# google-deepmind/mujoco_warp

Hardware: NVIDIA H100
Metric: env-steps/sec (whole box) on humanoid.xml at nworld=8192 per GPU (higher is better)
Workload: dtype f32

## Files before the change

mujoco_warp_b200/csrc/k_position.cu:

```cuda

#include "mjb_math.cuh"
#include "mjb_team.cuh"
#include "mjb_types.cuh"

namespace {

struct PosLayout {
  int qpos, xpos, xquat, xipos, xanchor, xaxis, scom, cinert, cdof, buf, arena, gxpos, gxmat, M, total;
};

__host__ __device__ inline int pad4(int n) { return (n + 3) & ~3; }
__host__ __device__ inline PosLayout pos_layout(const ModelDev& m) {
  PosLayout L;
  int o = 0;
  auto take = [&](int n) { int r = o; o += pad4(n); return r; };
  L.xpos = take(3 * m.nbody); L.xquat = take(4 * m.nbody); L.xipos = take(3 * m.nbody);
  L.xanchor = take(3 * m.njnt); L.xaxis = take(3 * m.njnt); L.scom = take(3 * m.nbody);
  L.arena = take(pad4(m.nq) > pad4(9 * m.nbody) ? m.nq : 9 * m.nbody);
  L.qpos = L.arena;
  L.gxpos = L.xipos; L.gxmat = L.gxpos + pad4(3 * m.ngeom);
  L.buf = L.xpos; L.M = L.buf + pad4(6 * m.nv);
  if (o < L.gxmat + pad4(9 * m.ngeom)) o = L.gxmat + pad4(9 * m.ngeom);
  if (o < L.M + pad4(m.nC)) o = L.M + pad4(m.nC);
  L.cinert = take(10 * m.nbody); L.cdof = take(6 * m.nv);
// ... 44 lines not shown
    __syncwarp();
#pragma unroll 1
    for (int l = 1; l < m.nlevel; l++) {
#pragma unroll 1
      for (int i = m.level_adr[l] + sub; i < m.level_adr[l + 1]; i += LPW) {
        const int b = m.level_body[i], pid = m.body_parentid[b], jntadr = m.body_jntadr[b], jntnum = m.body_jntnum[b];
        if (jntnum == 1 && m.jnt_type[jntadr] == JNT_FREE) {
          const int qa = m.jnt_qposadr[jntadr];
          v3 p = ld3(qpos + qa);
          q4 q = qnormalize(ldq(qpos + qa + 3));
          st3(xpos + 3 * b, p); stq(xquat + 4 * b, q);
          st3(xanchor + 3 * jntadr, p); st3(xaxis + 3 * jntadr, ld3(m.jnt_axis + 3 * jntadr));
          continue;
        }
        q4 pq = ldq(xquat + 4 * pid);
        const int mc = m.nmocap > 0 ? m.body_mocapid[b] : -1;
        const v3 bpos = mc >= 0 ? ld3(d.mocap_pos + (wb * m.nmocap + mc) * 3) : ld3(m.body_pos + 3 * b);
        const q4 bquat = mc >= 0 ? ldq(d.mocap_quat + (wb * m.nmocap + mc) * 4) : ldq(m.body_quat + 4 * b);
        v3 pos = qrot(pq, bpos) + ld3(xpos + 3 * pid);
        q4 quat = qmul(pq, bquat);
#pragma unroll 1
        for (int j = jntadr; j < jntadr + jntnum; j++) {
          const int qa = m.jnt_qposadr[j], t = m.jnt_type[j];
          v3 jpos = ld3(m.jnt_pos + 3 * j), jax = ld3(m.jnt_axis + 3 * j);
          v3 anchor = qrot(quat, jpos) + pos, axis = qrot(quat, jax);
          if (t == JNT_BALL) {
            quat = qmul(quat, qnormalize(ldq(qpos + qa)));
            pos = anchor - qrot(quat, jpos);
          } else if (t == JNT_SLIDE) {
            pos = pos + axis * (qpos[qa] - m.qpos0[qa]);
          } else if (t == JNT_HINGE) {
            quat = qmul(quat, axis_angle_quat(jax, qpos[qa] - m.qpos0[qa]));
            pos = anchor - qrot(quat, jpos);
          }
          st3(xanchor + 3 * j, anchor); st3(xaxis + 3 * j, axis);
        }
        st3(xpos + 3 * b, pos); stq(xquat + 4 * b, qnormalize(quat));
      }
      __syncwarp();
    }
  }

  if (kin && m.ntendon > 0) {
#pragma unroll 1
    for (int t = valid ? sub : m.ntendon; t < m.ntendon; t += LPW) {
      d.ten_length[wb * m.ntendon + t] = tendon_length(m, t, qpos);
      for (int k = m.ten_J_rowadr[t]; k < m.ten_J_rowadr[t] + m.ten_J_rownnz[t]; k++) d.ten_J[wb * m.nJten + k] = m.ten_J0[k];
    }
  }

  if (mask & STG_TRANSMISSION) {
#pragma unroll 1
    for (int a = valid ? sub : m.nu; a < m.nu; a += LPW) {
      if (m.ntendon > 0 && m.actuator_trntype[a] == TRN_TENDON) {
        const int t = m.actuator_trnid[2 * a], adr = m.moment_rowadr0[a], nnz = m.moment_rownnz0[a], tadr = m.ten_J_rowadr[t];
        const float gear0 = m.actuator_gear[6 * a];
        d.actuator_length[wb * m.nu + a] = tendon_length(m, t, qpos) * gear0;
        d.moment_rownnz[wb * m.nu + a] = nnz;
        d.moment_rowadr[wb * m.nu + a] = adr;
        for (int k = 0; k < nnz; k++) {
          d.moment_colind[wb * m.nJmom + adr + k] = m.moment_colind0[adr + k];
          d.actuator_moment[wb * m.nJmom + adr + k] = m.ten_J0[tadr + k] * gear0;
        }
        continue;
      }
      const int j = m.actuator_trnid[2 * a], t = m.jnt_type[j], adr = m.moment_rowadr0[a], nnz = m.moment_rownnz0[a];
      const float* gear = m.actuator_gear + 6 * a;
      d.actuator_length[wb * m.nu + a] = (t == JNT_SLIDE || t == JNT_HINGE) ? qpos[m.jnt_qposadr[j]] * gear[0] : 0.f;
      d.moment_rownnz[wb * m.nu + a] = nnz;
      d.moment_rowadr[wb * m.nu + a] = adr;
#pragma unroll 1
      for (int k = 0; k < nnz; k++) {
        d.moment_colind[wb * m.nJmom + adr + k] = m.moment_colind0[adr + k];
        d.actuator_moment[wb * m.nJmom + adr + k] = gear[k];
      }
    }
  }

  __syncwarp();

  if (kin) {
#pragma unroll 2
    for (int b = sub; b < nb; b += LPW) {
      q4 q = ldq(xquat + 4 * b);
      quat_to_mat(q, xmat + 9 * b);
      st3(xipos + 3 * b, ld3(xpos + 3 * b) + qrot(q, ld3(m.body_ipos + 3 * b)));
    }
#pragma unroll 1
    for (int s = valid ? sub : m.nsite; s < m.nsite; s += LPW) {
      const int b = m.site_bodyid[s];
      q4 q = ldq(xquat + 4 * b);
      float mat[9];
      st3(d.site_xpos + (wb * m.nsite + s) * 3, ld3(xpos + 3 * b) + qrot(q, ld3(m.site_pos + 3 * s)));
      quat_to_mat(qmul(q, ldq(m.site_quat + 4 * s)), mat);
      for (int k = 0; k < 9; k++) d.site_xmat[(wb * m.nsite + s) * 9 + k] = mat[k];
    }
    st.store_fence();
    GSTORE(xpos, BLK(xpos), 3 * nb); GSTORE(xquat, BLK(xquat), 4 * nb); GSTORE(xmat, BLK(arena), 9 * nb); GSTORE(xipos, BLK(xipos), 3 * nb);
    GSTORE(xanchor, BLK(xanchor), 3 * nj); GSTORE(xaxis, BLK(xaxis), 3 * nj);
    st.store_commit();
    if (!com) {
      st.store_wait_read();
#pragma unroll 2
      for (int b = sub; b < nb; b += LPW) quat_to_mat(qmul(ldq(xquat + 4 * b), ldq(m.body_iquat + 4 * b)), ximat + 9 * b);
      st.store_fence();
      GSTORE(ximat, BLK(arena), 9 * nb);
      st.store_commit();
    }
  }
  __syncwarp();

  if (com) {
#pragma unroll 2
    for (int b = sub; b < nb; b += LPW) st3(scom + 3 * b, ld3(xipos + 3 * b) * m.body_mass[b]);
    __syncwarp();
#pragma unroll 1
    for (int l = m.nlevel - 2; l >= 0; l--) {
#pragma unroll 1
      for (int i = m.level_adr[l] + sub; i < m.level_adr[l + 1]; i += LPW) {
        const int b = m.level_body[i];
        v3 acc = ld3(scom + 3 * b);
        for (int c = m.body_childadr[b]; c < m.body_childadr[b + 1]; c++) acc = acc + ld3(scom + 3 * m.body_childid[c]);
        st3(scom + 3 * b, acc);
      }
      __syncwarp();
    }
#pragma unroll 2
    for (int b = sub; b < nb; b += LPW) {
      const float ms = m.body_subtreemass[b];
      if (ms != 0.f) st3(scom + 3 * b, ld3(scom + 3 * b) * (1.0f / ms));
    }
    __syncwarp();
    if (kin) st.store_wait_read();
#pragma unroll 2
    for (int b = sub; b < nb; b += LPW) {
      float* mat = ximat + 9 * b;
      quat_to_mat(qmul(ldq(xquat + 4 * b), ldq(m.body_iquat + 4 * b)), mat);
      const v3 inert = ld3(m.body_inertia + 3 * b);
      const float mass = m.body_mass[b];
      const v3 dif = ld3(xipos + 3 * b) - ld3(scom + 3 * m.body_rootid[b]);
      float* r = cinert + 10 * b;
      const float a0 = mat[0] * inert.x, a1 = mat[1] * inert.y, a2 = mat[2] * inert.z;
      const float b0 = mat[3] * inert.x, b1 = mat[4] * inert.y, b2 = mat[5] * inert.z;
      const float c0 = mat[6] * inert.x, c1 = mat[7] * inert.y, c2 = mat[8] * inert.z;
      r[0] = a0 * mat[0] + a1 * mat[1] + a2 * mat[2] + mass * (dif.y * dif.y + dif.z * dif.z);
      r[1] = b0 * mat[3] + b1 * mat[4] + b2 * mat[5] + mass * (dif.x * dif.x + dif.z * dif.z);
      r[2] = c0 * mat[6] + c1 * mat[7] + c2 * mat[8] + mass * (dif.x * dif.x + dif.y * dif.y);
      r[3] = a0 * mat[3] + a1 * mat[4] + a2 * mat[5] - mass * dif.x * dif.y;
      r[4] = a0 * mat[6] + a1 * mat[7] + a2 * mat[8] - mass * dif.x * dif.z;
      r[5] = b0 * mat[6] + b1 * mat[7] + b2 * mat[8] - mass * dif.y * dif.z;
      r[6] = mass * dif.x; r[7] = mass * dif.y; r[8] = mass * dif.z; r[9] = mass;
    }
#pragma unroll 2
    for (int j = sub; j < nj; j += LPW) {
      const int b = m.jnt_bodyid[j], t = m.jnt_type[j];
      int dof = m.jnt_dofadr[j];
      const v3 offset = ld3(scom + 3 * m.body_rootid[b]) - ld3(xanchor + 3 * j);
      if (t == JNT_FREE || t == JNT_BALL) {
        float xm[9];
        quat_to_mat(ldq(xquat + 4 * b), xm);
        if (t == JNT_FREE) {
          for (int k = 0; k < 18; k++) cdof[6 * dof + k] = 0.f;
          cdof[6 * dof + 3] = 1.f; cdof[6 * (dof + 1) + 4] = 1.f; cdof[6 * (dof + 2) + 5] = 1.f;
          dof += 3;
        }
        for (int k = 0; k < 3; k++) {
          v3 col = matcol(xm, k);
          st3(cdof + 6 * (dof + k), col); st3(cdof + 6 * (dof + k) + 3, cross(col, offset));
        }
      } else if (t == JNT_SLIDE) {
        st3(cdof + 6 * dof, mk3(0.f, 0.f, 0.f)); st3(cdof + 6 * dof + 3, ld3(xaxis + 3 * j));
      } else {
        v3 ax = ld3(xaxis + 3 * j);
        st3(cdof + 6 * dof, ax); st3(cdof + 6 * dof + 3, cross(ax, offset));
      }
    }
    st.store_fence();
    GSTORE(subtree_com, BLK(scom), 3 * nb); GSTORE(cinert, BLK(cinert), 10 * nb); GSTORE(cdof, BLK(cdof), 6 * nv);
    if (kin) GSTORE(ximat, BLK(arena), 9 * nb);
    st.store_commit();
  }
  __syncwarp();

  if (mask & STG_CAMLIGHT) {
#pragma unroll 1
    for (int c = valid ? sub : m.ncam; c < m.ncam; c += LPW) {
      const int mode = m.cam_mode[c], b = m.cam_bodyid[c], tb = m.cam_targetbodyid[c];
      const bool is_target = mode == CAM_TARGETBODY || mode == CAM_TARGETBODYCOM;
      v3 p; float mat[9];
      if (mode == CAM_TRACK) {
        for (int k = 0; k < 9; k++) mat[k] = m.cam_mat0[9 * c + k];
        p = ld3(xpos + 3 * b) + ld3(m.cam_pos0 + 3 * c);
      } else if (mode == CAM_TRACKCOM) {
        for (int k = 0; k < 9; k++) mat[k] = m.cam_mat0[9 * c + k];
        p = ld3(scom + 3 * b) + ld3(m.cam_poscom0 + 3 * c);
      } else if (is_target && tb >= 0) {
        q4 q = ldq(xquat + 4 * b);
        p = ld3(xpos + 3 * b) + qrot(q, ld3(m.cam_pos + 3 * c));
        v3 tp = mode == CAM_TARGETBODYCOM ? ld3(scom + 3 * tb) : ld3(xpos + 3 * tb);
        v3 m3 = normalize(p - tp), m1 = normalize(cross(mk3(0.f, 0.f, 1.f), m3)), m2 = normalize(cross(m3, m1));
        mat[0] = m1.x; mat[1] = m2.x; mat[2] = m3.x; mat[3] = m1.y; mat[4] = m2.y; mat[5] = m3.y; mat[6] = m1.z; mat[7] = m2.z; mat[8] = m3.z;
      } else {
        q4 q = ldq(xquat + 4 * b);
        p = ld3(xpos + 3 * b) + qrot(q, ld3(m.cam_pos + 3 * c));
        quat_to_mat(qmul(q, ldq(m.cam_quat + 4 * c)), mat);
      }
      st3(d.cam_xpos + (wb * m.ncam + c) * 3, p);
      for (int k = 0; k < 9; k++) d.cam_xmat[(wb * m.ncam + c) * 9 + k] = mat[k];
    }
#pragma unroll 1
    for (int l = valid ? sub : m.nlight; l < m.nlight; l += LPW) {
      const int mode = m.light_mode[l], b = m.light_bodyid[l], tb = m.light_targetbodyid[l];
      const bool is_target = mode == CAM_TARGETBODY || mode == CAM_TARGETBODYCOM;
      v3 p, dir;
      bool norm = true;
      q4 q = ldq(xquat + 4 * b);
      if (is_target && tb < 0) {
        p = ld3(xpos + 3 * b) + qrot(q, ld3(m.light_pos + 3 * l)); dir = qrot(q, ld3(m.light_dir + 3 * l)); norm = false;
      } else if (mode == CAM_TRACK) {
        dir = ld3(m.light_dir0 + 3 * l); p = ld3(xpos + 3 * b) + ld3(m.light_pos0 + 3 * l);
      } else if (mode == CAM_TRACKCOM) {
        dir = ld3(m.light_dir0 + 3 * l); p = ld3(scom + 3 * b) + ld3(m.light_poscom0 + 3 * l);
      } else if (is_target) {
        p = ld3(xpos + 3 * b) + qrot(q, ld3(m.light_pos + 3 * l));
        v3 tp = mode == CAM_TARGETBODYCOM ? ld3(scom + 3 * tb) : ld3(xpos + 3 * tb);
        dir = tp - p;
      } else {
        p = ld3(xpos + 3 * b) + qrot(q, ld3(m.light_pos + 3 * l)); dir = qrot(q, ld3(m.light_dir + 3 * l));
      }
      if (norm) dir = normalize(dir);
      st3(d.light_xpos + (wb * m.nlight + l) * 3, p);
      st3(d.light_xdir + (wb * m.nlight + l) * 3, dir);
    }
  }


  if (kin) {
    st.store_wait_read();
#pragma unroll 2
    for (int gi = sub; gi < ng; gi += LPW) {
      const int b = m.geom_bodyid[gi];
      if (m.body_weldid[b] == 0 && (m.nmocap == 0 || m.body_mocapid[m.body_rootid[b]] == -1)) {
        for (int k = 0; k < 3; k++) gxpos[3 * gi + k] = d.geom_xpos[(wb * ng + gi) * 3 + k];
        for (int k = 0; k < 9; k++) gxmat[9 * gi + k] = d.geom_xmat[(wb * ng + gi) * 9 + k];
      } else {
        q4 q = ldq(xquat + 4 * b);
        st3(gxpos + 3 * gi, ld3(xpos + 3 * b) + qrot(q, ld3(m.geom_pos + 3 * gi)));
        quat_to_mat(qmul(q, ldq(m.geom_quat + 4 * gi)), gxmat + 9 * gi);
      }
    }
    st.store_fence();
    GSTORE(geom_xpos, BLK(gxpos), 3 * ng); GSTORE(geom_xmat, BLK(gxmat), 9 * ng);
    st.store_commit();
  }

  if (crbm) {
    st.store_wait_read();
#pragma unroll 1
    for (int l = m.nlevel - 2; l >= 1; l--) {
#pragma unroll 1
      for (int i = m.level_adr[l] + sub; i < m.level_adr[l + 1]; i += LPW) {
        const int b = m.level_body[i];
        float acc[10];
#pragma unroll
        for (int k = 0; k < 10; k++) acc[k] = crb[10 * b + k];
#pragma unroll 1
        for (int c = m.body_childadr[b]; c < m.body_childadr[b + 1]; c++) {
          const float* cc = crb + 10 * m.body_childid[c];
#pragma unroll
          for (int k = 0; k < 10; k++) acc[k] += cc[k];
        }
#pragma unroll
        for (int k = 0; k < 10; k++) crb[10 * b + k] = acc[k];
      }
      __syncwarp();
    }
#pragma unroll 2
    for (int dd = sub; dd < nv; dd += LPW) inert_vec(crb + 10 * m.dof_bodyid[dd], cdof + 6 * dd, buf + 6 * dd);
    __syncwarp();
#pragma unroll 4
    for (int e = sub; e < m.nC; e += LPW) {
      const int i = m.M_entry_row[e], j = m.M_colind[e];
      float v = dot6(cdof + 6 * j, buf + 6 * i);
      if (i == j) v += m.dof_armature[i];
      Ms[e] = v;
    }
    st.store_fence();
    GSTORE(crb, BLK(cinert), 10 * nb); GSTORE(M, BLK(M), m.nC);
    st.store_commit();
  }
  st.store_wait_read();
#undef GLOAD
#undef GSTORE
#undef BLK
#undef ROW
}

}

static TeamKernel pos_kernel(const ModelDev& m, int lpw) {
  return m.batched ? k_position<32, true> : lpw == 8 ? k_position<8, false> : lpw == 16 ? k_position<16, false> : k_position<32, false>;
}

size_t smem_position(const ModelDev& m, const DataDev& d) { return team_shape(m, d.wn, pos_layout(m).total, pos_kernel).block_bytes; }
cudaError_t launch_position(const ModelDev& m, const DataDev& d, int mask, cudaStream_t s) { return team_launch(m, d, pos_layout(m).total, pos_kernel, mask, s); }
cudaError_t resident_worlds_position(const ModelDev& m, const DataDev& d, int* worlds, int* shape) {
  shape[3] = 0;
  return team_resident_worlds(m, d, pos_layout(m).total, pos_kernel, worlds, shape);
}
```

mujoco_warp_b200/csrc/k_velocity.cu:

```cuda

#include "mjb_fluid.cuh"
#include "mjb_math.cuh"
#include "mjb_team.cuh"
#include "mjb_types.cuh"

namespace {

struct VelLayout { int qvel, cdof, cinert, cvel, cdofdot, cacc, cfrc, qpas, qbias, qact, qsm, qld, x, af, total; };
__host__ __device__ inline VelLayout vel_layout(const ModelDev& m) {
  VelLayout L;
  int o = 0;
  auto pad = [](int n) { return (n + 3) & ~3; };
  auto take = [&](int n) { int r = o; o += pad(n); return r; };
  L.qpas = take(m.nv); L.qbias = take(m.nv);
  L.qsm = L.qpas; L.x = L.qbias;
  const int a0 = o;
  L.cdof = take(6 * m.nv); L.cinert = take(10 * m.nbody); L.qvel = take(m.nv);
  L.cvel = take(6 * m.nbody); L.cdofdot = take(6 * (m.nv > m.nbody ? m.nv : m.nbody)); L.cacc = take(6 * m.nbody);
  L.cfrc = L.cdofdot;
  if (pad(m.nv) + pad(m.nu) <= L.cvel - L.cinert) { L.qact = L.cinert; L.af = L.cinert + pad(m.nv); }
  else { L.qact = take(m.nv); L.af = take(m.nu); }
  L.qld = a0;
  if (o - a0 < pad(m.qld_total)) o = a0 + pad(m.qld_total);
  L.total = o;
  return L;
}

template <int LPW>
__device__ __forceinline__ void team_chol_upper(float* U, int n, float* x, bool solve, int sub) {
#pragma unroll 1
  for (int j = 0; j < n; j++) {
    const int iend = solve ? n + 1 : n;
#pragma unroll 1
    for (int i = j + sub; i < iend; i += LPW) {
      const bool rhs = i == n;
      const float* col = rhs ? x : U + i;
      const int cs = rhs ? 1 : n;
      float s0 = rhs ? x[j] : U[j * n + i], s1 = 0.f;
      int k = 0;
#pragma unroll 4
      for (; k + 1 < j; k += 2) {
        s0 -= U[k * n + j] * col[k * cs];
        s1 -= U[(k + 1) * n + j] * col[(k + 1) * cs];
      }
      if (k < j) s0 -= U[k * n + j] * col[k * cs];
      if (rhs) x[j] = s0 + s1; else U[j * n + i] = s0 + s1;
    }
    __syncwarp();
    const float piv = sqrtf(fmaxf(U[j * n + j], MJ_MINVAL)), inv = 1.0f / piv;
    __syncwarp();
#pragma unroll 1
    for (int i = j + sub; i < iend; i += LPW) {
      if (i == n) x[j] *= inv;
      else U[j * n + i] = i == j ? piv : U[j * n + i] * inv;
    }
    __syncwarp();
  }
  if (!solve) return;
#pragma unroll 1
  for (int j = n - 1; j >= 0; j--) {
    const float xj = x[j] / U[j * n + j];
    __syncwarp();
#pragma unroll 1
    for (int k = sub; k < j; k += LPW) x[k] -= U[k * n + j] * xj;
    if (sub == 0) x[j] = xj;
    __syncwarp();
  }
}

template <bool PEXT, int LPW, bool BAT>
__global__ void __launch_bounds__(256)
k_velocity(const __grid_constant__ ModelDev mp, const __grid_constant__ DataDev d, int mask) {
  constexpr bool FLUID = false;
  [[maybe_unused]] constexpr FluidDev f{};
#include "k_velocity_body.cuh"
}

template <int LPW, bool BAT>
__global__ void __launch_bounds__(256)
k_velocity_fluid(const __grid_constant__ ModelDev mp, const __grid_constant__ DataDev d, int mask, const __grid_constant__ FluidDev f) {
  constexpr bool PEXT = true, FLUID = true;
#include "k_velocity_body.cuh"
}

}

template <bool PEXT>
static TeamKernel vel_instance(int lpw, bool bat) {
  if (bat) return k_velocity<PEXT, 32, true>;
  return lpw == 8 ? k_velocity<PEXT, 8, false> : lpw == 16 ? k_velocity<PEXT, 16, false> : k_velocity<PEXT, 32, false>;
}
static bool vel_pext(const ModelDev& m) { return m.has_gravcomp || m.ntendon > 0; }
static TeamKernel vel_kernel(const ModelDev& m, int lpw) { return vel_pext(m) ? vel_instance<true>(lpw, m.batched) : vel_instance<false>(lpw, m.batched); }
using FluidKernel = void (*)(ModelDev, DataDev, int, FluidDev);
static FluidKernel vel_kernel_fluid(const ModelDev& m, int lpw) {
  if (m.batched) return k_velocity_fluid<32, true>;
  return lpw == 8 ? k_velocity_fluid<8, false> : lpw == 16 ? k_velocity_fluid<16, false> : k_velocity_fluid<32, false>;
}

size_t smem_velocity(const ModelDev& m, const DataDev& d, const FluidDev& f) {
  const int words = vel_layout(m).total;
  return f.has_fluid ? team_shape(m, d.wn, words, vel_kernel_fluid).block_bytes : team_shape(m, d.wn, words, vel_kernel).block_bytes;
}
cudaError_t launch_velocity(const ModelDev& m, const DataDev& d, int mask, cudaStream_t s, const FluidDev& f) {
  const int words = vel_layout(m).total;
  return f.has_fluid ? team_launch(m, d, words, vel_kernel_fluid, mask, s, f) : team_launch(m, d, words, vel_kernel, mask, s);
}
cudaError_t resident_worlds_velocity(const ModelDev& m, const DataDev& d, int* worlds, int* shape, const FluidDev& f) {
  const int words = vel_layout(m).total;
  shape[3] = f.has_fluid ? 2 : vel_pext(m) ? 1 : 0;
  return f.has_fluid ? team_resident_worlds(m, d, words, vel_kernel_fluid, worlds, shape) : team_resident_worlds(m, d, words, vel_kernel, worlds, shape);
}
```

mujoco_warp_b200/csrc/k_velocity_body.cuh:

```cuda
  extern __shared__ __align__(16) float smem[];
  constexpr int G = 32 / LPW;
  Team<LPW> T;
  T.init(d.w0, d.wn, d.nworld);
  if (T.nvalid <= 0) return;
  MJB_WORLD_MODEL(T.w)
  const int lane = T.lane, sub = T.sub, g = T.g, nval = T.nvalid;
  const bool valid = T.valid;
  const VelLayout L = vel_layout(mp);
  float* S = smem + (size_t)(threadIdx.x >> 5) * ((size_t)L.total * G + 4);
  Stager st;
  st.init(reinterpret_cast<uint64_t*>(S + (size_t)L.total * G), lane);
  const int nv = m.nv, nb = m.nbody, nu = m.nu;
#define FLD(f, n) (S + (size_t)L.f * G + (size_t)g * (n))
  float *qvel = FLD(qvel, nv), *cdof = FLD(cdof, 6 * nv), *cinert = FLD(cinert, 10 * nb), *cvel = FLD(cvel, 6 * nb), *cdofdot = FLD(cdofdot, 6 * nv),
        *cacc = FLD(cacc, 6 * nb), *cfrc = FLD(cfrc, 6 * nb), *q_passive = FLD(qpas, nv), *q_bias = FLD(qbias, nv), *q_act = FLD(qact, nv),
        *q_smooth = FLD(qsm, nv), *qld = FLD(qld, m.qld_total), *x = FLD(x, nv), *aforce = FLD(af, nu);
  const float* Mw = d.M + (size_t)T.w * m.nC;
#undef FLD
  const size_t wg = (size_t)T.wg0;
#define GLOAD(f, field, n) st.load(S + (size_t)L.f * G, d.field + wg * (size_t)(n), nval * (n))
#define GSTORE(field, f, n) st.store(d.field + wg * (size_t)(n), S + (size_t)L.f * G, nval * (n))
  const size_t wb = (size_t)T.w;
  const bool v_all = mask & STG_VELOCITY;

  GLOAD(qvel, qvel, nv); GLOAD(cdof, cdof, 6 * nv);
  if (v_all || (mask & STG_RNE)) GLOAD(cinert, cinert, 10 * nb);
  constexpr int MREG = 32;
  float mreg[MREG];
  const bool fac = mask & (STG_ACCELERATION | STG_FACTOR_ONLY);
#pragma unroll
  for (int k = 0; k < MREG; k++) { const int e = sub + k * LPW; mreg[k] = (fac && e < m.nC) ? Mw[e] : 0.f; }
  bool any_xfrc = false;
  if (mask & STG_ACCELERATION) {
#pragma unroll 4
    for (int i = sub; i < 6 * nb; i += LPW) any_xfrc |= d.xfrc_applied[wb * 6 * nb + i] != 0.f;
  }
  st.load_wait();

  if (mask & (STG_VELOCITY | STG_COMVEL | STG_PASSIVE | STG_RNE)) {
    if (v_all)
#pragma unroll 1
    for (int a = valid ? sub : nu; a < nu; a += LPW) {
      const int nnz = d.moment_rownnz[wb * nu + a], adr = d.moment_rowadr[wb * nu + a];
      float vel = 0.f;
      for (int k = 0; k < nnz; k++) vel += d.actuator_moment[wb * m.nJmom + adr + k] * qvel[d.moment_colind[wb * m.nJmom + adr + k]];
      d.actuator_velocity[wb * nu + a] = vel;
    }
    if (PEXT && v_all && m.ntendon > 0) {
#pragma unroll 1
      for (int t = valid ? sub : m.ntendon; t < m.ntendon; t += LPW) {
        float vel = 0.f;
        for (int k = m.ten_J_rowadr[t]; k < m.ten_J_rowadr[t] + m.ten_J_rownnz[t]; k++) vel += m.ten_J0[k] * qvel[m.ten_J_colind[k]];
        d.ten_velocity[wb * m.ntendon + t] = vel;
      }
    }
    if (v_all || (mask & STG_COMVEL)) {
    if (sub < 6) cvel[sub] = 0.f;
    __syncwarp();
#pragma unroll 1
    for (int l = 1; l < m.nlevel; l++) {
#pragma unroll 1
      for (int i = m.level_adr[l] + sub; i < m.level_adr[l + 1]; i += LPW) {
        const int b = m.level_body[i], pid = m.body_parentid[b], jntadr = m.body_jntadr[b], jntnum = m.body_jntnum[b];
        int dof = m.body_dofadr[b];
        float cv[6];
#pragma unroll
        for (int k = 0; k < 6; k++) cv[k] = cvel[6 * pid + k];
#pragma unroll 1
        for (int j = jntadr; j < jntadr + jntnum; j++) {
          const int t = m.jnt_type[j];
          if (t == JNT_FREE) {
            for (int q = 0; q < 3; q++) { const float v = qvel[dof + q]; for (int k = 0; k < 6; k++) { cv[k] += cdof[6 * (dof + q) + k] * v; cdofdot[6 * (dof + q) + k] = 0.f; } }
            for (int q = 3; q < 6; q++) motion_cross(cv, cdof + 6 * (dof + q), cdofdot + 6 * (dof + q));
            for (int q = 3; q < 6; q++) { const float v = qvel[dof + q]; for (int k = 0; k < 6; k++) cv[k] += cdof[6 * (dof + q) + k] * v; }
            dof += 6;
          } else if (t == JNT_BALL) {
            for (int q = 0; q < 3; q++) motion_cross(cv, cdof + 6 * (dof + q), cdofdot + 6 * (dof + q));
            for (int q = 0; q < 3; q++) { const float v = qvel[dof + q]; for (int k = 0; k < 6; k++) cv[k] += cdof[6 * (dof + q) + k] * v; }
            dof += 3;
          } else {
            motion_cross(cv, cdof + 6 * dof, cdofdot + 6 * dof);
            const float v = qvel[dof];
            for (int k = 0; k < 6; k++) cv[k] += cdof[6 * dof + k] * v;
            dof += 1;
          }
        }
#pragma unroll
        for (int k = 0; k < 6; k++) cvel[6 * b + k] = cv[k];
      }
      __syncwarp();
    }
    st.store_fence();
    GSTORE(cvel, cvel, 6 * nb); GSTORE(cdof_dot, cdofdot, 6 * nv);
    st.store_commit();
    } else if (mask & STG_RNE) {
      GLOAD(cvel, cvel, 6 * nb); GLOAD(cdofdot, cdof_dot, 6 * nv);
      st.load_wait();
    }

    if (v_all || (mask & STG_PASSIVE)) {
      const bool dsbl_spring = m.disableflags & DSBL_SPRING, dsbl_damper = m.disableflags & DSBL_DAMPER;
      const bool gravcomp = PEXT && m.has_gravcomp && !(m.disableflags & DSBL_GRAVITY) && !(dsbl_spring && dsbl_damper);
      [[maybe_unused]] const bool fluid = FLUID && !(dsbl_spring && dsbl_damper);
      if constexpr (FLUID) if (fluid) {
        const float* cv = (v_all || (mask & STG_COMVEL)) ? cvel : d.cvel + wb * 6 * nb;
        const float *xip = d.xipos + wb * nb * 3, *stc = d.subtree_com + wb * nb * 3;
#pragma unroll 1
        for (int b = sub; b < nb; b += LPW)
          fluid_body_wrench(m, f, b, cv + 6 * b, ld3(xip + 3 * b), d.ximat + (wb * nb + b) * 9, ld3(stc + 3 * m.body_rootid[b]), d.geom_xpos + wb * m.ngeom * 3,
                            d.geom_xmat + wb * m.ngeom * 9, cacc + 6 * b);
        __syncwarp();
      }
#pragma unroll 1
      for (int dd = sub; dd < nv; dd += LPW) {
        const int j = m.dof_jntid[dd], t = m.jnt_type[j];
        float spring = 0.f, damper = 0.f, gc = 0.f;
        if (!(dsbl_spring && dsbl_damper)) {
          const float stiffness = m.jnt_stiffness[j];
          if (stiffness != 0.f && !dsbl_spring) {
            const int qa = m.jnt_qposadr[j], k = dd - m.jnt_dofadr[j];
            if (t == JNT_SLIDE || t == JNT_HINGE) spring = -(d.qpos[wb * m.nq + qa] - m.qpos_spring[qa]) * stiffness;
            else if (!PEXT) {}
            else if (t == JNT_FREE && k < 3) spring = -stiffness * (d.qpos[wb * m.nq + qa + k] - m.qpos_spring[qa + k]);
            else {
              const int ra = t == JNT_FREE ? qa + 3 : qa, kk = t == JNT_FREE ? k - 3 : k;
              const q4 rot = qnormalize(ldq(d.qpos + wb * m.nq + ra)), ref = ldq(m.qpos_spring + ra);
              const q4 qd = qmul(mkq(ref.w, -ref.x, -ref.y, -ref.z), rot);
              const float s2 = sqrtf(qd.x * qd.x + qd.y * qd.y + qd.z * qd.z);
              if (s2 != 0.f) {
                float speed = 2.0f * atan2f(s2, qd.w);
                if (speed > 3.14159265358979f) speed -= 2.0f * 3.14159265358979f;
                spring = -stiffness * (kk == 0 ? qd.x : kk == 1 ? qd.y : qd.z) * (speed / s2);
              }
            }
          }
          const float damping = m.dof_damping[dd];
          if (damping != 0.f && !dsbl_damper) damper = -qvel[dd] * damping;
          if (PEXT && m.ntendon > 0) {
#pragma unroll 1
            for (int tn = 0; tn < m.ntendon; tn++) {
              const float ks = m.tendon_stiffness[tn], kd = m.tendon_damping[tn];
              if ((ks == 0.f || dsbl_spring) && (kd == 0.f || dsbl_damper)) continue;
              const float J = tendon_J_at(m, tn, dd);
              if (J == 0.f) continue;
              if (ks != 0.f && !dsbl_spring) {
                const float len = d.ten_length[wb * m.ntendon + tn], lo = m.tendon_lengthspring[2 * tn], hi = m.tendon_lengthspring[2 * tn + 1];
                const float x = len > hi ? len - hi : (len < lo ? len - lo : 0.f);
                spring += J * (-x * ks);
              }
              if (kd != 0.f && !dsbl_damper) {
                float vel = 0.f;
                for (int k = m.ten_J_rowadr[tn]; k < m.ten_J_rowadr[tn] + m.ten_J_rownnz[tn]; k++) vel += m.ten_J0[k] * qvel[m.ten_J_colind[k]];
                damper += J * (-vel * kd);
              }
            }
          }
        }
        if (gravcomp) {
#pragma unroll 1
          for (int b = 1; b < nb; b++) {
            const float g = m.body_gravcomp[b];
            if (g == 0.f || !m.body_isdofancestor[b * nv + dd]) continue;
            const float sc = -m.body_mass[b] * g;
            const v3 off = ld3(d.xipos + (wb * nb + b) * 3) - ld3(d.subtree_com + (wb * nb + m.body_rootid[b]) * 3);
            const v3 jp = ld3(cdof + 6 * dd + 3) + cross(ld3(cdof + 6 * dd), off);
            gc += sc * (jp.x * m.gravity_x + jp.y * m.gravity_y + jp.z * m.gravity_z);
          }
        }
        float passive = spring + damper + (m.jnt_actgravcomp[j] ? 0.f : gc);
        if constexpr (FLUID) {
          const float fl = fluid ? fluid_project(m, dd, cdof + 6 * dd, cacc, d.xipos + wb * nb * 3, d.subtree_com + wb * nb * 3) : 0.f;
          passive += fl;
          if (valid) f.qfrc_fluid[wb * nv + dd] = fl;
        }
        q_passive[dd] = passive;
        if (valid) {
          d.qfrc_spring[wb * nv + dd] = spring;
          d.qfrc_damper[wb * nv + dd] = damper;
          d.qfrc_gravcomp[wb * nv + dd] = gc;
          d.qfrc_passive[wb * nv + dd] = passive;
        }
      }
    }
    if (v_all || (mask & STG_RNE)) {
    for (int k = sub; k < 6; k += LPW) cacc[k] = k < 3 ? 0.f : ((m.disableflags & DSBL_GRAVITY) ? 0.f : -(k == 3 ? m.gravity_x : k == 4 ? m.gravity_y : m.gravity_z));
    __syncwarp();
#pragma unroll 1
    for (int l = 1; l < m.nlevel; l++) {
#pragma unroll 1
      for (int i = m.level_adr[l] + sub; i < m.level_adr[l + 1]; i += LPW) {
        const int b = m.level_body[i], pid = m.body_parentid[b];
        float a[6];
#pragma unroll
        for (int k = 0; k < 6; k++) a[k] = cacc[6 * pid + k];
#pragma unroll 1
        for (int q = 0; q < m.body_dofnum[b]; q++) {
          const int dof = m.body_dofadr[b] + q;
          const float v = qvel[dof];
#pragma unroll
          for (int k = 0; k < 6; k++) a[k] += cdofdot[6 * dof + k] * v;
        }
#pragma unroll
        for (int k = 0; k < 6; k++) cacc[6 * b + k] = a[k];
      }
      __syncwarp();
    }
    st.store_wait_read();
#pragma unroll 2
    for (int b = sub; b < nb; b += LPW) {
      float f[6] = {0.f, 0.f, 0.f, 0.f, 0.f, 0.f};
      if (b > 0) {
        float iv[6], g[6];
        inert_vec(cinert + 10 * b, cacc + 6 * b, f);
        inert_vec(cinert + 10 * b, cvel + 6 * b, iv);
        motion_cross_force(cvel + 6 * b, iv, g);
#pragma unroll
        for (int k = 0; k < 6; k++) f[k] += g[k];
      }
#pragma unroll
      for (int k = 0; k < 6; k++) cfrc[6 * b + k] = f[k];
    }
    __syncwarp();
#pragma unroll 1
    for (int l = m.nlevel - 2; l >= 0; l--) {
#pragma unroll 1
      for (int i = m.level_adr[l] + sub; i < m.level_adr[l + 1]; i += LPW) {
        const int b = m.level_body[i];
        float acc[6];
#pragma unroll
        for (int k = 0; k < 6; k++) acc[k] = cfrc[6 * b + k];
#pragma unroll 1
        for (int c = m.body_childadr[b]; c < m.body_childadr[b + 1]; c++) {
          const float* cc = cfrc + 6 * m.body_childid[c];
#pragma unroll
          for (int k = 0; k < 6; k++) acc[k] += cc[k];
        }
#pragma unroll
        for (int k = 0; k < 6; k++) cfrc[6 * b + k] = acc[k];
      }
      __syncwarp();
    }
#pragma unroll 1
    for (int dd = sub; dd < nv; dd += LPW) {
      const float v = dot6(cdof + 6 * dd, cfrc + 6 * m.dof_bodyid[dd]);
      q_bias[dd] = v;
    }
    st.store_fence();
    GSTORE(cacc, cacc, 6 * nb); GSTORE(cfrc_int, cfrc, 6 * nb); GSTORE(qfrc_bias, qbias, nv);
    st.store_commit();
    }
  } else if (mask & STG_ACCELERATION) {
    GLOAD(qpas, qfrc_passive, nv); GLOAD(qbias, qfrc_bias, nv);
    st.load_wait();
  }
  __syncwarp();

  if (mask & STG_ACTUATION) {
#pragma unroll 1
    for (int dd = sub; dd < nv; dd += LPW) q_act[dd] = 0.f;
    __syncwarp();
    const bool enabled = nu > 0 && !(m.disableflags & DSBL_ACTUATION);
#pragma unroll 1
    for (int a = sub; a < nu; a += LPW) {
      float force = 0.f;
      if (enabled) {
        float ctrl = d.ctrl[wb * nu + a];
        if (m.actuator_ctrllimited[a] && !(m.disableflags & DSBL_CLAMPCTRL)) ctrl = clampf(ctrl, m.actuator_ctrlrange[2 * a], m.actuator_ctrlrange[2 * a + 1]);
        const float length = d.actuator_length[wb * nu + a], velocity = d.actuator_velocity[wb * nu + a];
        const float *gp = m.actuator_gainprm + 10 * a, *bp = m.actuator_biasprm + 10 * a;
        float gain = 0.f, bias = 0.f;
        if (m.actuator_gaintype[a] == GAIN_FIXED) gain = gp[0];
        else if (m.actuator_gaintype[a] == GAIN_AFFINE) gain = gp[0] + gp[1] * length + gp[2] * velocity;
        if (m.actuator_biastype[a] == BIAS_AFFINE) bias = bp[0] + bp[1] * length + bp[2] * velocity;
        float ctrl_act = ctrl;
        if (m.na > 0 && m.actuator_actadr[a] >= 0) {
          const int last = m.actuator_actadr[a] + m.actuator_actnum[a] - 1, dyn = m.actuator_dyntype[a];
          const float act = d.act[wb * m.na + last];
          float act_dot = 0.f;
          if (dyn == DYN_INTEGRATOR) act_dot = ctrl;
          else if (dyn == DYN_FILTER || dyn == DYN_FILTEREXACT) act_dot = (ctrl - act) / fmaxf(m.actuator_dynprm[10 * a], MJ_MINVAL);
          if (valid) d.act_dot[wb * m.na + last] = act_dot;
          ctrl_act = m.actuator_actearly[a] ? next_act(m, a, act, act_dot, 1.0f, m.actuator_actlimited[a] != 0) : act;
        }
        force = gain * ctrl_act + bias;
        if (m.actuator_forcelimited[a]) force = clampf(force, m.actuator_forcerange[2 * a], m.actuator_forcerange[2 * a + 1]);
      } else if (m.na > 0 && m.actuator_actadr[a] >= 0 && valid) {
        d.act_dot[wb * m.na + m.actuator_actadr[a] + m.actuator_actnum[a] - 1] = 0.f;
      }
      if (valid) d.actuator_force[wb * nu + a] = force;
      aforce[a] = force;
    }
    __syncwarp();
    if (PEXT && enabled && m.ntendon > 0) {
#pragma unroll 1
      for (int t = sub; t < m.ntendon; t += LPW) {
        if (!m.tendon_actfrclimited[t]) continue;
        float total = 0.f;
        for (int b = 0; b < nu; b++) if (m.actuator_trntype[b] == TRN_TENDON && m.actuator_trnid[2 * b] == t) total += aforce[b];
        const float lo = m.tendon_actfrcrange[2 * t], hi = m.tendon_actfrcrange[2 * t + 1];
        const float sc = total < lo ? lo / total : (total > hi ? hi / total : 1.0f);
        if (sc == 1.0f) continue;
        for (int b = 0; b < nu; b++)
          if (m.actuator_trntype[b] == TRN_TENDON && m.actuator_trnid[2 * b] == t) { aforce[b] *= sc; if (valid) d.actuator_force[wb * nu + b] = aforce[b]; }
      }
      __syncwarp();
    }
    if (enabled) {
#pragma unroll 1
      for (int dd = sub; dd < nv; dd += LPW) {
        float q = 0.f;
        for (int k = m.dofact_adr[dd]; k < m.dofact_adr[dd + 1]; k++) q += d.actuator_moment[wb * m.nJmom + m.dofact_mom[k]] * aforce[m.dofact_act[k]];
        const int j = m.dof_jntid[dd];
        if (!(m.disableflags & DSBL_GRAVITY) && m.jnt_actgravcomp[j]) q += d.qfrc_gravcomp[wb * nv + dd];
        if (m.jnt_actfrclimited[j]) q = clampf(q, m.jnt_actfrcrange[2 * j], m.jnt_actfrcrange[2 * j + 1]);
        q_act[dd] = q;
      }
    }
    st.store_fence();
    GSTORE(qfrc_actuator, qact, nv);
    st.store_commit();
  } else if (mask & STG_ACCELERATION) {
    GLOAD(qact, qfrc_actuator, nv);
    st.load_wait();
  }
  __syncwarp();

  if (mask & (STG_ACCELERATION | STG_FACTOR_ONLY)) {
    if (mask & STG_ACCELERATION) {
#pragma unroll 1
      for (int dd = sub; dd < nv; dd += LPW) q_smooth[dd] = q_passive[dd] - q_bias[dd] + q_act[dd] + d.qfrc_applied[wb * nv + dd];
      if (team_any<LPW>(any_xfrc, g)) {
#pragma unroll 1
        for (int dd = sub; dd < nv; dd += LPW) {
          const float* cd = cdof + 6 * dd;
          const int db = m.dof_bodyid[dd];
          float acc = 0.f;
          for (int b = db; b < nb; b++) {
            const float* ft = d.xfrc_applied + (wb * nb + b) * 6;
            if (ft[0] == 0.f && ft[1] == 0.f && ft[2] == 0.f && ft[3] == 0.f && ft[4] == 0.f && ft[5] == 0.f) continue;
            int p = b;
            while (p != 0 && p != db) p = m.body_parentid[p];
            if (p == 0) continue;
            const v3 off = ld3(d.xipos + (wb * nb + b) * 3) - ld3(d.subtree_com + (wb * nb + m.body_rootid[b]) * 3);
            const v3 cr = cross(ld3(cd), off);
            acc += cd[3] * ft[0] + cd[4] * ft[1] + cd[5] * ft[2] + cd[0] * ft[3] + cd[1] * ft[4] + cd[2] * ft[5] + dot(cr, ld3(ft));
          }
          q_smooth[dd] += acc;
        }
      }
      __syncwarp();
    }
    const bool acc = mask & STG_ACCELERATION;
    st.store_wait_read();
#pragma unroll 1
    for (int i = sub; i < m.qld_total; i += LPW) qld[i] = 0.f;
    if (acc)
#pragma unroll 1
      for (int i = sub; i < nv; i += LPW) x[i] = q_smooth[i];
    __syncwarp();
#pragma unroll 1
    for (int t = 0; t < m.ntree; t++) {
      const int start = m.tree_dofadr[t], n = m.tree_dofnum[t];
      float* U = qld + m.tree_qLDadr[t];
      const int e0 = m.M_rowadr[start], e1 = m.M_rowadr[start + n - 1] + m.M_rownnz[start + n - 1];
#pragma unroll
      for (int k = 0; k < MREG; k++) {
        const int e = sub + k * LPW;
        if (e >= e0 && e < e1) U[(m.M_colind[e] - start) * n + (m.M_entry_row[e] - start)] = mreg[k];
      }
#pragma unroll 1
      for (int e = max(e0, MREG * LPW) + ((sub - max(e0, MREG * LPW)) % LPW + LPW) % LPW; e < e1; e += LPW)
        U[(m.M_colind[e] - start) * n + (m.M_entry_row[e] - start)] = Mw[e];
      __syncwarp();
      team_chol_upper<LPW>(U, n, x + start, acc, sub);
    }
    st.store_fence();
    if (acc) { GSTORE(qfrc_smooth, qsm, nv); GSTORE(qacc_smooth, x, nv); }
    GSTORE(qLD, qld, m.qld_total);
    st.store_commit();
  }
  st.store_wait_read();
#undef GLOAD
#undef GSTORE
```

mujoco_warp_b200/csrc/mjb_team.cuh:

```cuda
#pragma once
#include <algorithm>
#include <climits>
#include <cstdint>
#include <cuda_runtime.h>

#include "mjb_launch.cuh"
#include "mjb_math.cuh"
#include "mjb_types.cuh"

template <int LPW>
__device__ __forceinline__ float team_sum(float v) {
#pragma unroll
  for (int o = LPW / 2; o > 0; o >>= 1) v += __shfl_xor_sync(FULL_MASK, v, o);
  return v;
}
template <int LPW>
__device__ __forceinline__ int team_sum_i(int v) {
#pragma unroll
  for (int o = LPW / 2; o > 0; o >>= 1) v += __shfl_xor_sync(FULL_MASK, v, o);
  return v;
}
template <int LPW>
__device__ __forceinline__ bool team_any(bool p, int g) {
  const unsigned b = __ballot_sync(FULL_MASK, p);
  return LPW == 32 ? b != 0u : ((b >> (g * LPW)) & ((1u << (LPW & 31)) - 1u)) != 0u;
}

__device__ __forceinline__ uint32_t smem_u32(const void* p) { return (uint32_t)__cvta_generic_to_shared(p); }

struct Stager {
  uint64_t* bar;
  uint32_t phase;
  int lane;
  bool pending_store;

  __device__ __forceinline__ void init(uint64_t* b, int lane_) {
    bar = b; phase = 0; lane = lane_; pending_store = false;
    if (lane == 0) {
      asm volatile("mbarrier.init.shared::cta.b64 [%0], 1;" ::"r"(smem_u32(bar)) : "memory");
      asm volatile("fence.mbarrier_init.release.cluster;" ::: "memory");
    }
    __syncwarp();
  }
  static __device__ __forceinline__ bool bulk_ok(const void* g, const void* s, int nfloats) {
    return (((uintptr_t)g | (uintptr_t)smem_u32(s)) & 15u) == 0 && (nfloats & 3) == 0 && nfloats > 0;
  }
  __device__ __forceinline__ void load(float* s, const float* g, int n) {
    if (bulk_ok(g, s, n)) {
      if (lane == 0) {
        const uint32_t bytes = (uint32_t)n * 4u;
        asm volatile("mbarrier.expect_tx.relaxed.cta.shared::cta.b64 [%0], %1;" ::"r"(smem_u32(bar)), "r"(bytes) : "memory");
        asm volatile("cp.async.bulk.shared::cluster.global.mbarrier::complete_tx::bytes [%0], [%1], %2, [%3];" ::"r"(smem_u32(s)), "l"(g),
                     "r"(bytes), "r"(smem_u32(bar))
                     : "memory");
      }
    } else {
#pragma unroll 1
      for (int i = lane; i < n; i += 32) s[i] = g[i];
    }
  }
  __device__ __forceinline__ void load_wait() {
    if (lane == 0) asm volatile("mbarrier.arrive.shared::cta.b64 _, [%0];" ::"r"(smem_u32(bar)) : "memory");
    uint32_t ok = 0;
    while (!ok) {
      asm volatile("{\n .reg .pred p;\n mbarrier.try_wait.parity.shared::cta.b64 p, [%1], %2;\n selp.u32 %0, 1, 0, p;\n}" : "=r"(ok) : "r"(smem_u32(bar)), "r"(phase) : "memory");
    }
    phase ^= 1u;
    __syncwarp();
  }
  __device__ __forceinline__ void store_fence() {
    asm volatile("fence.proxy.async.shared::cta;" ::: "memory");
    __syncwarp();
  }
  __device__ __forceinline__ void store(float* g, const float* s, int n) {
    if (bulk_ok(g, s, n)) {
      if (lane == 0) {
        asm volatile("cp.async.bulk.global.shared::cta.bulk_group [%0], [%1], %2;" ::"l"(g), "r"(smem_u32(s)), "r"((uint32_t)n * 4u) : "memory");
        pending_store = true;
      }
    } else {
#pragma unroll 1
      for (int i = lane; i < n; i += 32) g[i] = s[i];
    }
  }
  __device__ __forceinline__ void store_commit() {
    if (lane == 0 && pending_store) asm volatile("cp.async.bulk.commit_group;" ::: "memory");
  }
  __device__ __forceinline__ void store_wait_read() {
    if (lane == 0 && pending_store) { asm volatile("cp.async.bulk.wait_group.read 0;" ::: "memory"); pending_store = false; }
    __syncwarp();
  }
};

using TeamKernel = void (*)(ModelDev, DataDev, int);
template <class K>
using TeamChooserOf = K (*)(const ModelDev& m, int lpw);

struct TeamShape { int lpw, wpb; size_t block_bytes; };
template <class K>
inline TeamShape team_shape(const ModelDev& m, int nworld, size_t world_words, TeamChooserOf<K> kernel_of) {
  constexpr size_t kBlockMax = 200 * 1024;
  auto bytes = [&](int lpw) { return (world_words * (size_t)(32 / lpw) + 4) * sizeof(float); };
  int lpw = 8;
  while (lpw < 32 && bytes(lpw) > kBlockMax / 2) lpw *= 2;
  int wpb = 2;
  if (m.batched && lpw < 32) {
    lpw = 32;
  } else {
    const SmLimits& sm = sm_limits();
    const long groups = (nworld + 32 / lpw - 1) / (32 / lpw);
    const int warp_regs = (kernel_regs(kernel_of(m, lpw)) * 32 + 255) & ~255;
    auto rounds = [&](int w) {
      long per_sm = (long)(sm.smem_per_sm / sm_block_bytes(bytes(lpw) * w));
      per_sm = std::min({per_sm, (long)sm.blocks, (long)(sm.warps / w)});
      if (warp_regs > 0) per_sm = std::min(per_sm, (long)(sm.regs / warp_regs / w));
      const long fit = per_sm * sm.sms, blocks = (groups + w - 1) / w;
      return fit > 0 ? (blocks + fit - 1) / fit : LONG_MAX;
    };
    for (int w : {1, 4})
      if (bytes(lpw) * w <= kBlockMax && rounds(w) < rounds(wpb)) wpb = w;
  }
  while (wpb > 1 && bytes(lpw) * wpb > kBlockMax) wpb--;
  return TeamShape{lpw, wpb, bytes(lpw) * wpb};
}

inline int team_carveout(size_t block_bytes) {
  const size_t per_sm = sm_limits().smem_per_sm, block = sm_block_bytes(block_bytes), fit = per_sm / block;
  const size_t pct = fit > 0 ? (100 * fit * block + per_sm - 1) / per_sm : 100;
  return pct < 100 ? (int)pct : (int)cudaSharedmemCarveoutMaxShared;
}

template <class K, class... A>
inline cudaError_t team_launch(const ModelDev& m, const DataDev& d, size_t world_words, TeamChooserOf<K> kernel_of, int mask, cudaStream_t s, const A&... extra) {
  const TeamShape t = team_shape(m, d.wn, world_words, kernel_of);
  const int G = 32 / t.lpw, ngroups = (d.wn + G - 1) / G, grid = (ngroups + t.wpb - 1) / t.wpb;
  return launch(kernel_of(m, t.lpw), grid, 32 * t.wpb, t.block_bytes, team_carveout(t.block_bytes), s, m, d, mask, extra...);
}

template <class K>
inline cudaError_t team_resident_worlds(const ModelDev& m, const DataDev& d, size_t world_words, TeamChooserOf<K> kernel_of, int* worlds, int* shape) {
  const TeamShape t = team_shape(m, d.wn, world_words, kernel_of);
  const K kern = kernel_of(m, t.lpw);
  int blocks = 0;
  cudaError_t e = launch_configure((const void*)kern, t.block_bytes, team_carveout(t.block_bytes));
  if (e == cudaSuccess) e = cudaOccupancyMaxActiveBlocksPerMultiprocessor(&blocks, kern, 32 * t.wpb, t.block_bytes);
  *worlds = blocks * t.wpb * (32 / t.lpw);
  shape[0] = t.lpw; shape[1] = t.wpb; shape[2] = (int)t.block_bytes;
  return e;
}

template <int LPW>
struct Team {
  static constexpr int G = 32 / LPW;
  int lane, sub, g;
  int wg0, nvalid;
  int w;
  bool valid;
  __device__ __forceinline__ void init(int w0, int wn, int nworld) {
    lane = threadIdx.x & 31; sub = lane % LPW; g = lane / LPW;
    wg0 = w0 + (blockIdx.x * (blockDim.x >> 5) + (threadIdx.x >> 5)) * G;
    const int wend = min(w0 + wn, nworld);
    nvalid = min(G, wend - wg0);
    valid = g < nvalid;
    w = wg0 + (valid ? g : nvalid - 1);
  }
};
```

Measured before the change: 20.71 million.

## Let velocity kernel pick wider lanes-per-world teams with shifted bulk copies

The launch shape search now considers wider lane-per-world teams (up to the model's max tree size) for the velocity kernel when they need no more scheduling rounds. It also sizes from the total world count instead of the per-launch slice. To keep bulk async copies usable when per-world blocks are not 16-byte aligned at two worlds per warp, shared buffers are offset to match global alignment, with shifted load/store helpers that handle the unaligned edges. The LPW=16 instantiation gets a tighter launch bound and a smaller register array for the mass matrix, trading register spills for occupancy.

Result: faster. 20.91 million (median of 6 runs) (+1.0%).

```diff
diff --git a/mujoco_warp_b200/csrc/k_position.cu b/mujoco_warp_b200/csrc/k_position.cu
--- a/mujoco_warp_b200/csrc/k_position.cu
+++ b/mujoco_warp_b200/csrc/k_position.cu
@@ -370,9 +370,9 @@
   return m.batched ? k_position<32, true> : lpw == 8 ? k_position<8, false> : lpw == 16 ? k_position<16, false> : k_position<32, false>;
 }
 
-size_t smem_position(const ModelDev& m, const DataDev& d) { return team_shape(m, d.wn, pos_layout(m).total, pos_kernel).block_bytes; }
-cudaError_t launch_position(const ModelDev& m, const DataDev& d, int mask, cudaStream_t s) { return team_launch(m, d, pos_layout(m).total, pos_kernel, mask, s); }
+size_t smem_position(const ModelDev& m, const DataDev& d) { return team_shape(m, d.nworld, pos_layout(m).total, pos_kernel, 0).block_bytes; }
+cudaError_t launch_position(const ModelDev& m, const DataDev& d, int mask, cudaStream_t s) { return team_launch(m, d, pos_layout(m).total, pos_kernel, 0, mask, s); }
 cudaError_t resident_worlds_position(const ModelDev& m, const DataDev& d, int* worlds, int* shape) {
   shape[3] = 0;
-  return team_resident_worlds(m, d, pos_layout(m).total, pos_kernel, worlds, shape);
-}
+  return team_resident_worlds(m, d, pos_layout(m).total, pos_kernel, 0, worlds, shape);
+}
diff --git a/mujoco_warp_b200/csrc/k_velocity.cu b/mujoco_warp_b200/csrc/k_velocity.cu
--- a/mujoco_warp_b200/csrc/k_velocity.cu
+++ b/mujoco_warp_b200/csrc/k_velocity.cu
@@ -69,7 +69,7 @@
 }
 
 template <bool PEXT, int LPW, bool BAT>
-__global__ void __launch_bounds__(256)
+__global__ void __launch_bounds__(256, LPW == 16 ? 4 : 2)
 k_velocity(const __grid_constant__ ModelDev mp, const __grid_constant__ DataDev d, int mask) {
   constexpr bool FLUID = false;
   [[maybe_unused]] constexpr FluidDev f{};
@@ -100,14 +100,14 @@
 
 size_t smem_velocity(const ModelDev& m, const DataDev& d, const FluidDev& f) {
   const int words = vel_layout(m).total;
-  return f.has_fluid ? team_shape(m, d.wn, words, vel_kernel_fluid).block_bytes : team_shape(m, d.wn, words, vel_kernel).block_bytes;
+  return f.has_fluid ? team_shape(m, d.nworld, words, vel_kernel_fluid, m.maxtree).block_bytes : team_shape(m, d.nworld, words, vel_kernel, m.maxtree).block_bytes;
 }
 cudaError_t launch_velocity(const ModelDev& m, const DataDev& d, int mask, cudaStream_t s, const FluidDev& f) {
   const int words = vel_layout(m).total;
-  return f.has_fluid ? team_launch(m, d, words, vel_kernel_fluid, mask, s, f) : team_launch(m, d, words, vel_kernel, mask, s);
+  return f.has_fluid ? team_launch(m, d, words, vel_kernel_fluid, m.maxtree, mask, s, f) : team_launch(m, d, words, vel_kernel, m.maxtree, mask, s);
 }
 cudaError_t resident_worlds_velocity(const ModelDev& m, const DataDev& d, int* worlds, int* shape, const FluidDev& f) {
   const int words = vel_layout(m).total;
   shape[3] = f.has_fluid ? 2 : vel_pext(m) ? 1 : 0;
-  return f.has_fluid ? team_resident_worlds(m, d, words, vel_kernel_fluid, worlds, shape) : team_resident_worlds(m, d, words, vel_kernel, worlds, shape);
+  return f.has_fluid ? team_resident_worlds(m, d, words, vel_kernel_fluid, m.maxtree, worlds, shape) : team_resident_worlds(m, d, words, vel_kernel, m.maxtree, worlds, shape);
 }
diff --git a/mujoco_warp_b200/csrc/k_velocity_body.cuh b/mujoco_warp_b200/csrc/k_velocity_body.cuh
--- a/mujoco_warp_b200/csrc/k_velocity_body.cuh
+++ b/mujoco_warp_b200/csrc/k_velocity_body.cuh
@@ -11,21 +11,22 @@
   Stager st;
   st.init(reinterpret_cast<uint64_t*>(S + (size_t)L.total * G), lane);
   const int nv = m.nv, nb = m.nbody, nu = m.nu;
-#define FLD(f, n) (S + (size_t)L.f * G + (size_t)g * (n))
+  const int wgi = T.wg0;
+#define BLK(f, n) (S + (size_t)L.f * G + team_shift<G>(wgi, n))
+#define FLD(f, n) (BLK(f, n) + (size_t)g * (n))
   float *qvel = FLD(qvel, nv), *cdof = FLD(cdof, 6 * nv), *cinert = FLD(cinert, 10 * nb), *cvel = FLD(cvel, 6 * nb), *cdofdot = FLD(cdofdot, 6 * nv),
         *cacc = FLD(cacc, 6 * nb), *cfrc = FLD(cfrc, 6 * nb), *q_passive = FLD(qpas, nv), *q_bias = FLD(qbias, nv), *q_act = FLD(qact, nv),
         *q_smooth = FLD(qsm, nv), *qld = FLD(qld, m.qld_total), *x = FLD(x, nv), *aforce = FLD(af, nu);
   const float* Mw = d.M + (size_t)T.w * m.nC;
-#undef FLD
   const size_t wg = (size_t)T.wg0;
-#define GLOAD(f, field, n) st.load(S + (size_t)L.f * G, d.field + wg * (size_t)(n), nval * (n))
-#define GSTORE(field, f, n) st.store(d.field + wg * (size_t)(n), S + (size_t)L.f * G, nval * (n))
+#define GLOAD(f, field, n) st.load_shifted(BLK(f, n), d.field + wg * (size_t)(n), nval * (n))
+#define GSTORE(field, f, n) st.store_shifted(d.field + wg * (size_t)(n), BLK(f, n), nval * (n))
   const size_t wb = (size_t)T.w;
   const bool v_all = mask & STG_VELOCITY;
 
   GLOAD(qvel, qvel, nv); GLOAD(cdof, cdof, 6 * nv);
   if (v_all || (mask & STG_RNE)) GLOAD(cinert, cinert, 10 * nb);
-  constexpr int MREG = 32;
+  constexpr int MREG = LPW == 16 ? 8 : 32;
   float mreg[MREG];
   const bool fac = mask & (STG_ACCELERATION | STG_FACTOR_ONLY);
 #pragma unroll
@@ -382,3 +383,5 @@
   st.store_wait_read();
 #undef GLOAD
 #undef GSTORE
+#undef FLD
+#undef BLK
diff --git a/mujoco_warp_b200/csrc/mjb_team.cuh b/mujoco_warp_b200/csrc/mjb_team.cuh
--- a/mujoco_warp_b200/csrc/mjb_team.cuh
+++ b/mujoco_warp_b200/csrc/mjb_team.cuh
@@ -28,6 +28,13 @@
 
 __device__ __forceinline__ uint32_t smem_u32(const void* p) { return (uint32_t)__cvta_generic_to_shared(p); }
 
+template <int G>
+__device__ __forceinline__ int team_shift(int wg0, int n) {
+  if (G != 2) return 0;
+  const int h = (int)(((size_t)wg0 * (size_t)n) & 3u);
+  return ((h + G * n + 3) & ~3) <= G * ((n + 3) & ~3) ? h : 0;
+}
+
 struct Stager {
   uint64_t* bar;
   uint32_t phase;
@@ -45,6 +52,9 @@
   static __device__ __forceinline__ bool bulk_ok(const void* g, const void* s, int nfloats) {
     return (((uintptr_t)g | (uintptr_t)smem_u32(s)) & 15u) == 0 && (nfloats & 3) == 0 && nfloats > 0;
   }
+  static __device__ __forceinline__ bool congruent(const void* g, const void* s) {
+    return ((uintptr_t)g & 3u) == 0 && (((uintptr_t)g - smem_u32(s)) & 15u) == 0;
+  }
   __device__ __forceinline__ void load(float* s, const float* g, int n) {
     if (bulk_ok(g, s, n)) {
       if (lane == 0) {
@@ -59,6 +69,32 @@
       for (int i = lane; i < n; i += 32) s[i] = g[i];
     }
   }
+  __device__ __forceinline__ void store(float* g, const float* s, int n) {
+    if (bulk_ok(g, s, n)) {
+      if (lane == 0) {
+        asm volatile("cp.async.bulk.global.shared::cta.bulk_group [%0], [%1], %2;" ::"l"(g), "r"(smem_u32(s)), "r"((uint32_t)n * 4u) : "memory");
+        pending_store = true;
+      }
+    } else {
+#pragma unroll 1
+      for (int i = lane; i < n; i += 32) g[i] = s[i];
+    }
+  }
+  __device__ __forceinline__ void load_shifted(float* s, const float* g, int n) {
+    if (n > 0 && congruent(g, s)) {
+      if (lane == 0) {
+        const int h = (int)(((uintptr_t)g >> 2) & 3u);
+        const uint32_t bytes = (uint32_t)((h + n + 3) & ~3) * 4u;
+        asm volatile("mbarrier.expect_tx.relaxed.cta.shared::cta.b64 [%0], %1;" ::"r"(smem_u32(bar)), "r"(bytes) : "memory");
+        asm volatile("cp.async.bulk.shared::cluster.global.mbarrier::complete_tx::bytes [%0], [%1], %2, [%3];" ::"r"(smem_u32(s - h)), "l"(g - h),
+                     "r"(bytes), "r"(smem_u32(bar))
+                     : "memory");
+      }
+    } else {
+#pragma unroll 1
+      for (int i = lane; i < n; i += 32) s[i] = g[i];
+    }
+  }
   __device__ __forceinline__ void load_wait() {
     if (lane == 0) asm volatile("mbarrier.arrive.shared::cta.b64 _, [%0];" ::"r"(smem_u32(bar)) : "memory");
     uint32_t ok = 0;
@@ -72,12 +108,14 @@
     asm volatile("fence.proxy.async.shared::cta;" ::: "memory");
     __syncwarp();
   }
-  __device__ __forceinline__ void store(float* g, const float* s, int n) {
-    if (bulk_ok(g, s, n)) {
-      if (lane == 0) {
-        asm volatile("cp.async.bulk.global.shared::cta.bulk_group [%0], [%1], %2;" ::"l"(g), "r"(smem_u32(s)), "r"((uint32_t)n * 4u) : "memory");
+  __device__ __forceinline__ void store_shifted(float* g, const float* s, int n) {
+    const int h = (int)(((16u - ((uintptr_t)g & 15u)) & 15u) >> 2), mid = (n - h) & ~3;
+    if (n - h >= 4 && congruent(g, s)) {
+      if (lane == 0) {
+        asm volatile("cp.async.bulk.global.shared::cta.bulk_group [%0], [%1], %2;" ::"l"(g + h), "r"(smem_u32(s + h)), "r"((uint32_t)mid * 4u) : "memory");
         pending_store = true;
       }
+      if (lane < n - mid) { const int i = lane < h ? lane : lane + mid; g[i] = s[i]; }
     } else {
 #pragma unroll 1
       for (int i = lane; i < n; i += 32) g[i] = s[i];
@@ -98,15 +136,13 @@
 
 struct TeamShape { int lpw, wpb; size_t block_bytes; };
 template <class K>
-inline TeamShape team_shape(const ModelDev& m, int nworld, size_t world_words, TeamChooserOf<K> kernel_of) {
+inline TeamShape team_shape(const ModelDev& m, int nworld, size_t world_words, TeamChooserOf<K> kernel_of, int loop_len) {
   constexpr size_t kBlockMax = 200 * 1024;
   auto bytes = [&](int lpw) { return (world_words * (size_t)(32 / lpw) + 4) * sizeof(float); };
-  int lpw = 8;
-  while (lpw < 32 && bytes(lpw) > kBlockMax / 2) lpw *= 2;
-  int wpb = 2;
-  if (m.batched && lpw < 32) {
-    lpw = 32;
-  } else {
+  int lpw0 = 8;
+  while (lpw0 < 32 && bytes(lpw0) > kBlockMax / 2) lpw0 *= 2;
+  struct Fit { int lpw, wpb; long rounds, blocks; };
+  auto shape_at = [&](int lpw) {
     const SmLimits& sm = sm_limits();
     const long groups = (nworld + 32 / lpw - 1) / (32 / lpw);
     const int warp_regs = (kernel_regs(kernel_of(m, lpw)) * 32 + 255) & ~255;
@@ -117,11 +153,20 @@
       const long fit = per_sm * sm.sms, blocks = (groups + w - 1) / w;
       return fit > 0 ? (blocks + fit - 1) / fit : LONG_MAX;
     };
-    for (int w : {1, 4})
-      if (bytes(lpw) * w <= kBlockMax && rounds(w) < rounds(wpb)) wpb = w;
-  }
-  while (wpb > 1 && bytes(lpw) * wpb > kBlockMax) wpb--;
-  return TeamShape{lpw, wpb, bytes(lpw) * wpb};
+    int wpb = 2;
+    if (!m.batched)
+      for (int w : {1, 4})
+        if (bytes(lpw) * w <= kBlockMax && rounds(w) < rounds(wpb)) wpb = w;
+    while (wpb > 1 && bytes(lpw) * wpb > kBlockMax) wpb--;
+    return Fit{lpw, wpb, rounds(wpb), (groups + wpb - 1) / wpb};
+  };
+  Fit best = shape_at(m.batched ? 32 : lpw0);
+  if (!m.batched && best.blocks >= sm_limits().sms)
+    for (int lpw = best.lpw * 2; lpw <= 32 && lpw < loop_len; lpw *= 2) {
+      const Fit f = shape_at(lpw);
+      if (f.rounds <= best.rounds) best = f;
+    }
+  return TeamShape{best.lpw, best.wpb, bytes(best.lpw) * best.wpb};
 }
 
 inline int team_carveout(size_t block_bytes) {
@@ -131,15 +176,17 @@
 }
 
 template <class K, class... A>
-inline cudaError_t team_launch(const ModelDev& m, const DataDev& d, size_t world_words, TeamChooserOf<K> kernel_of, int mask, cudaStream_t s, const A&... extra) {
-  const TeamShape t = team_shape(m, d.wn, world_words, kernel_of);
+inline cudaError_t team_launch(const ModelDev& m, const DataDev& d, size_t world_words, TeamChooserOf<K> kernel_of, int loop_len, int mask, cudaStream_t s,
+                               const A&... extra) {
+  const TeamShape t = team_shape(m, d.nworld, world_words, kernel_of, loop_len);
   const int G = 32 / t.lpw, ngroups = (d.wn + G - 1) / G, grid = (ngroups + t.wpb - 1) / t.wpb;
   return launch(kernel_of(m, t.lpw), grid, 32 * t.wpb, t.block_bytes, team_carveout(t.block_bytes), s, m, d, mask, extra...);
 }
 
 template <class K>
-inline cudaError_t team_resident_worlds(const ModelDev& m, const DataDev& d, size_t world_words, TeamChooserOf<K> kernel_of, int* worlds, int* shape) {
-  const TeamShape t = team_shape(m, d.wn, world_words, kernel_of);
+inline cudaError_t team_resident_worlds(const ModelDev& m, const DataDev& d, size_t world_words, TeamChooserOf<K> kernel_of, int loop_len, int* worlds,
+                                        int* shape) {
+  const TeamShape t = team_shape(m, d.nworld, world_words, kernel_of, loop_len);
   const K kern = kernel_of(m, t.lpw);
   int blocks = 0;
   cudaError_t e = launch_configure((const void*)kern, t.block_bytes, team_carveout(t.block_bytes));
```
